# nmonette/TO-UED

Measured on AMD Instinct MI355X. Metric: agent-env-steps/sec (inner rollout) at num_agents=512; meta-updates/sec, higher is better.
Workload: dtype f32; 1 GPU; C2 LPG meta-gradient env_mode=tabular num_agents=512 num_mini_batches=1 W=64 T=20 K=5 score_function=random; num_agents=512, agents_per_gpu=512, env_workers=64, train_rollout_len=20, num_agent_updates=5, parallelism=dp1 (agent axis)

## Files before the change

### include/toued.h

```cpp
#ifndef TOUED_H
#define TOUED_H

#include <stddef.h>
#include <stdint.h>

#ifdef __cplusplus
extern "C" {
#endif

typedef struct ihipStream_t* hipStream_t;

typedef struct {
  int max_grid;
  int n_max;
  int n_types;
  int tabular;
} EnvSpec;

const char* toued_last_error(void);
int toued_abi_version(void);

typedef struct toued_ctx toued_ctx;
toued_ctx* toued_ctx_create(void);
int toued_ctx_destroy(toued_ctx* ctx);
// ... 27 lines not shown
                  int* obs_idx, int* obs_time, float* reward, uint8_t* done, int n, hipStream_t stream);

int toued_batch_reset(EnvSpec spec, const int* levels, const uint32_t* agent_keys, int n_agents, int W, int* state,
                      int* obs_idx, int* obs_time, hipStream_t stream);
int toued_batch_reset_masked(EnvSpec spec, const int* levels, const uint32_t* agent_keys, int n_agents, int W,
                             int* state, int* obs_idx, int* obs_time, const uint8_t* mask, hipStream_t stream);
int toued_rollout(EnvSpec spec, const int* levels, const float* theta, int D, const uint32_t* agent_keys,
                  int* state, int n_agents, int W, int T, int* traj_idx, int* traj_time, uint8_t* traj_action,
                  float* traj_reward, uint8_t* traj_done, float* cum_return, hipStream_t stream);
int toued_rollout_draws(EnvSpec spec, const int* levels, const uint32_t* keys, int n_agents, int U, int W, int T,
                        uint32_t* chain, uint32_t* draws, hipStream_t stream);
int toued_rollout_env(EnvSpec spec, const int* levels, const float* theta, int D, int* state, int n_agents, int W, int T,
                      const uint32_t* draws, long dstride, int* traj_idx, int* traj_time, uint8_t* traj_action,
                      float* traj_reward, uint8_t* traj_done, float* cum_return, hipStream_t stream);
int toued_eval_keys(const uint32_t* agent_keys, int n_agents, int W, int T, uint32_t* chain, hipStream_t stream);
int toued_eval_draws(EnvSpec spec, const int* levels, int n_agents, int W, int T, const uint32_t* chain,
                     uint32_t* draws, hipStream_t stream);
int toued_eval_returns(EnvSpec spec, const int* levels, const float* theta, int D, const int* state, int n_agents,
                       int W, int T, const uint32_t* draws, float* cum_return, hipStream_t stream);
int toued_eval_returns_cus(int n_workers);
int toued_optimal_return(const int* levels, int n, int max_grid, int n_max, int tabular, int max_rollout_len,
                         float* v0, float* v_all, hipStream_t stream);
int toued_policy_return(const int* levels, const float* theta, int n, int D, int max_grid, int n_max, int tabular,
                        int max_rollout_len, float* v0, float* v_all, hipStream_t stream);
int toued_policy_return_moments(const int* levels, const float* theta, int n, int D, int max_grid, int n_max,
                                int tabular, int max_rollout_len, float* v0, float* var0, float* v_all,
                                float* var_all, hipStream_t stream);


int toued_choice_cdf(const uint32_t* key, const float* cdf, int B, int n, int* out, hipStream_t stream);
// ... 165 lines not shown
                           float* d_y_hat, hipStream_t stream);

int toued_agent_step_snap(int N, int W, int T, int D, float* theta, float* phi, const int* tidx, const int* ttime,
                          const uint8_t* tact, const float* trew, const uint8_t* tdone, const float* pi_hat,
                          const float* y_hat, float alpha_y, float lr_a, float lr_c, float max_norm, float* Gth,
                          float* Gph, float* met, int* step, const int* levels, float* gstat, float* snap_th0,
                          float* snap_ph0, float* snap_last0, float* snap_th1, float* snap_ph1, float* snap_last1,
                          hipStream_t stream);
int toued_entropy_clip_hvp_snap(int N, int W, int T, int D, int K, const float* snap_th1, const float* snap_ph1,
                                const float* snap_last1, const float* snap_th0, const float* snap_ph0,
                                const float* snap_last0, const int* tidx, const int* ttime, const uint8_t* tact,
                                const float* pi_hat, const float* y_hat, float coef_a, float coef_c, float* adj_th,
                                float* adj_ph, const float* Gth, const float* Gph, const float* gstat, float lr_a,
                                float lr_c, float max_norm, float* coef, float alpha_y, float b2, float b3,
                                float* d_pi_hat, float* d_y_hat, hipStream_t stream);
int toued_embed_bwd_snap(int N, int W, int T, int D, int K, const float* snap_ph, const float* snap_last,
                         const int* ttime_hist, long tidx_stride, const uint8_t* tdone_hist, long tstep_stride,
                         const float* dX3, const float* dX4, long dx_stride_k, const float* e1w, const float* e1b,
                         const float* e2w, float* partial, int n_blocks, hipStream_t stream);

int toued_gru_pack_fwd_multi(const float* eta, long eta_stride, int n, const int* off, int F, float* fwdA,
                             hipStream_t stream);
int toued_gru_fwd_multi(int R, int T, int W, int F, int rows_per_cand, const float* X, long xs_f, long xs_col,
                        const uint8_t* done, const float* fwdA, const float* eta, long eta_stride, const int* off,
                        float* pi_hat, float* y_hat, hipStream_t stream);

int toued_es_ask(const uint32_t* key, long nd, long half_pop, long row_lo, long n_rows, const float* mean,
                 float sigma, float* x, hipStream_t stream);
int toued_es_grad(const float* x, const float* mean, float sigma, const float* fitness, int C, long nd, float* out,
                  hipStream_t stream);
// ... 8 lines not shown
```

### to-ued_amd/csrc/agent.hip

```cpp
#include <string.h>
#include <algorithm>
#include <type_traits>
#include "common.h"
#include "wave_dev.h"

#define EPSF 1e-8f
#define SORT_MAX_TW 2048

namespace {

TOUED_DEV float wave_sum(float v) {
#pragma unroll
  for (int o = 32; o > 0; o >>= 1) v += __shfl_xor(v, o, 64);
  return v;
}

template <int K>
TOUED_DEV void probs_of(const float* __restrict__ tab, const float* __restrict__ last, int idx, float c, float* p) {
  float l[K];
  float m = -__builtin_inff();
#pragma unroll
  for (int j = 0; j < K; ++j) {
    l[j] = *reinterpret_cast<const float*>(reinterpret_cast<const char*>(tab) + ((unsigned)idx * K + j) * 4u) + c * last[j];
    m = fmaxf(m, l[j]);
// ... 561 lines not shown
  }
  __syncthreads();
  if (tid == 0) {
    met[a * 8 + 3] += (red[0][0] + red[0][1]) + (red[0][2] + red[0][3]);
    met[a * 8 + 4] += (red[1][0] + red[1][1]) + (red[1][2] + red[1][3]);
  }
}

__global__ void __launch_bounds__(256) k_entropy_metric(int W, int T, int D, const float* __restrict__ theta,
                                                        const float* __restrict__ phi, const int* __restrict__ tidx,
                                                        const int* __restrict__ ttime, float* __restrict__ met) {
  __shared__ float red[2][4];
  entropy_metric_agent(blockIdx.x, threadIdx.x, W, T, D, theta, phi, tidx, ttime, met, red);
}

__global__ void __launch_bounds__(64) k_eval_loss(int N, int W, int T, int D, const float* __restrict__ theta,
                                                  const float* __restrict__ vcrit, const int* __restrict__ tidx,
                                                  const int* __restrict__ ttime, const uint8_t* __restrict__ tact,
                                                  const float* __restrict__ trew, const uint8_t* __restrict__ tdone,
                                                  float gamma, float lam, float* __restrict__ adv_scratch,
                                                  float* __restrict__ abar, float* __restrict__ out) {
  const int a = blockIdx.x;
  const int lane = threadIdx.x;
  const float* v = vcrit + (size_t)a * D;
  const float vlast = v[D - 1];
  const float* th = theta + (size_t)a * D * 5;
  float lastA[5];
#pragma unroll
  for (int j = 0; j < 5; ++j) lastA[j] = th[(size_t)(D - 1) * 5 + j];
  float* adv = adv_scratch + (size_t)a * W * T;
  float s_adv = 0.0f, s_vl = 0.0f;
  for (int w = lane; w < W; w += 64) {
    float vn = v[tidx[((size_t)a * (T + 1) + T) * W + w]] + ((float)ttime[((size_t)a * (T + 1) + T) * W + w] * 0.001f) * vlast;
    float g = 0.0f, vl = 0.0f;
    for (int t = T - 1; t >= 0; --t) {
      const size_t o0 = ((size_t)a * (T + 1) + t) * W + w;
// ... 1263 lines not shown
  if (ROWS_PRIO > 0) __builtin_amdgcn_s_setprio(ROWS_PRIO);
  rows_sorted_body<Op, false>(op);
}

#ifndef ROWS2_WPE
#define ROWS2_WPE 4
#endif
template <class Op1, class Op2>
__global__ void __launch_bounds__(512) __attribute__((amdgpu_waves_per_eu(ROWS2_WPE))) k_rows_sorted2(Op1 op1, Op2 op2) {
  if (ROWS_PRIO > 0) __builtin_amdgcn_s_setprio(ROWS_PRIO);
  rows_sorted_body<Op1, false, 1>(op1);
  __syncthreads();
  rows_sorted_body<Op2, true, 2>(op2);
}

template <class Op>
static bool launch_sorted(const Op& op, int N, hipStream_t stream) {
  const int TW = op.T * op.W;
  if (TW > SORT_MAX_TW || TW <= 0 || op.D >= (1 << 20)) return false;
  const size_t bytes = 2048 * 4 + (size_t)TW * (Op::NA + Op::NC) * 4;
  static bool attr_set = false;
  if (!attr_set) {
    if (hipFuncSetAttribute(reinterpret_cast<const void*>(&k_rows_sorted<Op>),
                            hipFuncAttributeMaxDynamicSharedMemorySize, 120 * 1024) != hipSuccess)
      return false;
    attr_set = true;
  }
  hipLaunchKernelGGL(k_rows_sorted<Op>, dim3(N), dim3(512), bytes, stream, op);
  return true;
}
// ... 264 lines not shown
      EntropyBwdOpT<true>{snap_th1, snap_ph1, tidx, ttime, coef_a, coef_c, adj_th, adj_ph, N, W, T, D, snap_last1};
  ec.Gth = Gth;
  ec.Gph = Gph;
  ec.gstat = gstat;
  ec.lr_a = lr_a;
  ec.lr_c = lr_c;
  ec.max_norm = max_norm;
  ec.coef = coef;
  const HvpOpT<true> hv{snap_th0, snap_ph0, tidx, ttime, tact, pi_hat, y_hat, Gth, Gph, adj_th, adj_ph, coef, lr_a,
                        lr_c, alpha_y, b2, b3, adj_th, adj_ph, d_pi_hat, d_y_hat, N, W, T, D, K, snap_last0};
  TOUED_REQUIRE(launch_sorted2(ec, hv, N, stream), "toued_entropy_clip_hvp_snap: cannot launch the sorted kernel");
  TOUED_CHECK_LAUNCH();
  return 0;
}

int toued_agent_apply(int N, int D, const float* th0, const float* ph0, const float* Gth, const float* Gph,
                      float lr_a, float lr_c, float max_norm, int* step, float* th1, float* ph1, const float* gstat,
                      hipStream_t stream) {
  if (N == 0 || D == 0) return 0;
  const bool v4 = aligned16(th0) && aligned16(ph0) && aligned16(Gth) && aligned16(Gph) && aligned16(th1) &&
                  aligned16(ph1);
  const long nvec = v4 ? (long)D * 2 + 1 : (long)D * 8;
  const unsigned gx = (unsigned)std::max(1L, std::min(64L, (nvec + 511) / 512));
  hipLaunchKernelGGL(k_agent_apply, dim3(gx, N, 2), dim3(256), 0, stream, N, D, th0, ph0, Gth, Gph, lr_a, lr_c,
                     max_norm, step, th1, ph1, gstat, v4 ? 1 : 0);
  TOUED_CHECK_LAUNCH();
  return 0;
}

int toued_entropy(int N, int W, int T, int D, const float* theta, const float* phi, const int* tidx, const int* ttime,
// ... 181 lines not shown
```

### to-ued_amd/csrc/env.hip

```cpp
#include "env_dev.h"

#include <cstdlib>
#include <cstring>

namespace {

template <int NMAX, bool TAB>
__global__ void __launch_bounds__(256) k_gw_reset(EnvSpec sp, const int* __restrict__ levels, int W,
                                                  const uint32_t* __restrict__ keys, int* __restrict__ state,
                                                  int* __restrict__ obs_idx, int* __restrict__ obs_time, int n) {
  const int i = blockIdx.x * blockDim.x + threadIdx.x;
  if (i >= n) return;
  const int* lev = levels + (size_t)(i / W) * LEVEL_WORDS;
  EnvState s;
  reset_env<NMAX, TAB>(sp, lev, make_uint2(keys[2 * i], keys[2 * i + 1]), s);
  store_state<NMAX>(state, n, i, s);
  obs_idx[i] = tab_index(sp, s);
  obs_time[i] = s.time;
}

template <int NMAX, bool TAB>
__global__ void __launch_bounds__(256) k_gw_step(EnvSpec sp, const int* __restrict__ levels, int W,
                                                 const uint32_t* __restrict__ keys, int* __restrict__ state,
                                                 const int* __restrict__ actions, int* __restrict__ obs_idx,
// ... 161 lines not shown

__global__ void __launch_bounds__(256) k_eval_keys(const uint32_t* __restrict__ agent_keys, int W, int T, int n,
                                                   uint4* __restrict__ chain) {
  const int i = blockIdx.x * blockDim.x + threadIdx.x;
  if (i >= n) return;
  const int a = i / W, w = i - a * W;
  uint2 r = split_at(make_uint2(agent_keys[2 * a], agent_keys[2 * a + 1]), (uint32_t)W, (uint32_t)w);
  for (int t = 0; t < T; ++t) {
    uint2 sub, sub_env;
    split2(r, r, sub);
    split2(r, r, sub_env);
    chain[(size_t)t * n + i] = make_uint4(sub.x, sub.y, sub_env.x, sub_env.y);
  }
}

__global__ void __launch_bounds__(1024) k_eval_keys_pairs(const uint32_t* __restrict__ agent_keys, int W, int T, int n,
                                                         uint2* __restrict__ chain) {
  const int g = blockIdx.x * blockDim.x + threadIdx.x;
  const int i = g >> 1;
  const uint32_t j = (uint32_t)(g & 1);
  if (i >= n) return;
  const int a = i / W, w = i - a * W;
  uint2 r = split_at(make_uint2(agent_keys[2 * a], agent_keys[2 * a + 1]), (uint32_t)W, (uint32_t)w);
  auto xor1 = [](uint32_t v) { return (uint32_t)__builtin_amdgcn_update_dpp(0, (int)v, 0xB1, 0xF, 0xF, false); };
  auto split_pair = [&](uint2& key, uint2& sub) {
    const uint2 y = threefry(key.x, key.y, j, j + 2u);
    const uint32_t px = xor1(y.x), py = xor1(y.y);
    key = j ? make_uint2(px, y.x) : make_uint2(y.x, px);
    sub = j ? make_uint2(py, y.y) : make_uint2(y.y, py);
  };
  for (int t = 0; t < T; ++t) {
    uint2 sub, sub_env;
    split_pair(r, sub);
    split_pair(r, sub_env);
    chain[((size_t)t * n + i) * 2 + j] = j ? sub_env : sub;
  }
}

template <int NMAX>
__global__ void __launch_bounds__(256) k_eval_draws(const int* __restrict__ levels, int W, int na, int n, long total,
                                                    const uint4* __restrict__ chain, uint4* __restrict__ draws) {
  const long j = (long)blockIdx.x * blockDim.x + threadIdx.x;
  if (j >= total) return;
  const int i = (int)(j % n);
  const int* lev = levels + (size_t)((i / W) % na) * LEVEL_WORDS;
  const uint4 c = chain[j];
  const draw4 d = step_draws<NMAX>(lev, make_uint2(c.x, c.y), make_uint2(c.z, c.w));
  draws[j] = make_uint4(d.x, d.y, d.z, d.w);
}

#ifdef H3_PLACE
// ... 124 lines not shown
    s.pos = pos;
    s.exists = (s.exists | (int)dr.z) & ~collected & used;
    s.early_term = term;
  }
  cum_return[i] = cum;
  if (EVAL_CHOSEN_ROW == 2 && warm == 1.2345e-38f) cum_return[i] = warm;
#ifdef H3_PLACE
  if (threadIdx.x == 0 && blockIdx.x < 64) {
    const unsigned slot = g_evr_launch & 63u;
    g_evr_place[(slot * 64 + blockIdx.x) * 2] = (unsigned)__builtin_amdgcn_s_getreg((3 << 11) | 20);
    g_evr_place[(slot * 64 + blockIdx.x) * 2 + 1] = (unsigned)__builtin_amdgcn_s_getreg((31 << 11) | 4);
  }
#endif
}

template <int NMAX, bool CAND>
__global__ void __launch_bounds__(256) k_train_env(EnvSpec sp, const int* __restrict__ levels,
                                                   const float* __restrict__ theta, int D, int* __restrict__ state,
                                                   int T, int W, int n, const uint4* __restrict__ draws, long dstride,
                                                   int* __restrict__ traj_idx, int* __restrict__ traj_time,
                                                   uint8_t* __restrict__ traj_action, float* __restrict__ traj_reward,
                                                   uint8_t* __restrict__ traj_done, float* __restrict__ cum_return) {
  const int i = blockIdx.x * blockDim.x + threadIdx.x;
  if (i >= n) return;
  const int a = i / W, w = i - a * W;
  const float* tab = theta + (size_t)a * D * 5;
  TrainWorker<NMAX, CAND> wk;
  wk.init(sp, levels, a, theta, D, state, n, i);
  wk.load_rows(tab, D);
  float cum = 0.0f, valid = 1.0f;
  const size_t base_o = (size_t)a * (T + 1) * W + w, base_t = (size_t)a * T * W + w;
  const draw4* dw = reinterpret_cast<const draw4*>(draws);
  draw4 dr0 = {0u, 0u, 0u, 0u};
  if (T > 0) dr0 = dw[i];
  draw4 dr1 = dr0;
  if (T > 1) dr1 = dw[dstride + i];
  for (int t = 0; t < T; ++t) {
// ... 85 lines not shown
  return 0;
}

int toued_batch_reset_masked(EnvSpec sp, const int* levels, const uint32_t* agent_keys, int n_agents, int W, int* state,
                             int* obs_idx, int* obs_time, const uint8_t* mask, hipStream_t stream) {
  if (int e = check_spec(sp)) return e;
  TOUED_REQUIRE(n_agents >= 0 && W >= 1 && mask, "toued_batch_reset_masked: bad sizes N=%d W=%d", n_agents, W);
  const int n = n_agents * W;
  if (n == 0) return 0;
  TOUED_DISPATCH(sp, hipLaunchKernelGGL((k_batch_reset<NMAX, TAB>), dim3(nblk(n)), dim3(256), 0, stream, sp, levels,
                                        agent_keys, W, state, obs_idx, obs_time, n, mask));
  TOUED_CHECK_LAUNCH();
  return 0;
}

int toued_eval_keys(const uint32_t* agent_keys, int n_agents, int W, int T, uint32_t* chain, hipStream_t stream) {
  TOUED_REQUIRE(n_agents >= 0 && W >= 1 && T >= 0, "toued_eval_keys: bad sizes N=%d W=%d T=%d", n_agents, W, T);
  const int n = n_agents * W;
  if (n == 0 || T == 0) return 0;
  static const int kb = [] {
    const char* e = getenv("TOUED_EVAL_KEYS_BLOCK");
    return e ? atoi(e) : 64;
  }();
  hipLaunchKernelGGL(k_eval_keys_pairs, dim3((unsigned)((2L * n + kb - 1) / kb)), dim3(kb), 0, stream, agent_keys, W, T,
                     n, reinterpret_cast<uint2*>(chain));
  TOUED_CHECK_LAUNCH();
  return 0;
}

int toued_eval_draws(EnvSpec sp, const int* levels, int n_agents, int W, int T, const uint32_t* chain, uint32_t* draws,
                     hipStream_t stream) {
  if (int e = check_spec(sp)) return e;
  TOUED_REQUIRE(sp.tabular, "toued_eval_draws: tabular envs only");
  TOUED_REQUIRE(n_agents >= 0 && W >= 1 && T >= 0, "toued_eval_draws: bad sizes N=%d W=%d T=%d", n_agents, W, T);
  const int n = n_agents * W;
  const long total = (long)n * T;
  if (total == 0) return 0;
  const unsigned g = (unsigned)((total + 255) / 256);
  TOUED_DISPATCH_NMAX(sp.n_max, true, hipLaunchKernelGGL(k_eval_draws<NMAX>, dim3(g), dim3(256), 0, stream, levels,
                                                        W, n_agents, n, total, reinterpret_cast<const uint4*>(chain),
                                                        reinterpret_cast<uint4*>(draws)));
  TOUED_CHECK_LAUNCH();
// ... 125 lines not shown
```

### to-ued_amd/toued/_lib.py

```python
from __future__ import annotations

import ctypes
import os
from pathlib import Path

import torch

LIB_PATH = Path(os.environ.get("TOUED_LIB", Path(__file__).resolve().parent / "libtoued_hip.so"))


class ToUEDError(RuntimeError):
    pass


class EnvSpecC(ctypes.Structure):
    _fields_ = [("max_grid", ctypes.c_int), ("n_max", ctypes.c_int), ("n_types", ctypes.c_int),
                ("tabular", ctypes.c_int)]


_P = ctypes.c_void_p
_I = ctypes.c_int
_F = ctypes.c_float
_U = ctypes.c_uint32
_L = ctypes.c_long
# ... 3 lines not shown
    "toued_split_planar": [_P, _I, _I, _P, _P],
    "toued_fold_in": [_P, _I, _U, _P, _P],
    "toued_random_bits": [_P, _I, _I, _P, _P],
    "toued_uniform": [_P, _I, _I, _F, _F, _P, _P],
    "toued_normal": [_P, _I, _I, _P, _P],
    "toued_mode_program_bytes": [],
    "toued_level_gen": [_P, _P, _P, _P, _P, _I, _P],
    "toued_level_gen_masked": [_P, _P, _P, _P, _I, _P, _P],
    "toued_level_edit": [_P, _P, _P, _I, _I, _I, _F, _I, _I, _F, _P, _P, _P],
    "toued_gw_reset": [EnvSpecC, _P, _I, _P, _P, _P, _P, _I, _P],
    "toued_gw_step": [EnvSpecC, _P, _I, _P, _P, _P, _P, _P, _P, _P, _I, _P],
    "toued_batch_reset": [EnvSpecC, _P, _P, _I, _I, _P, _P, _P, _P],
    "toued_batch_reset_masked": [EnvSpecC, _P, _P, _I, _I, _P, _P, _P, _P, _P],
    "toued_rollout": [EnvSpecC, _P, _P, _I, _P, _P, _I, _I, _I, _P, _P, _P, _P, _P, _P, _P],
    "toued_eval_keys": [_P, _I, _I, _I, _P, _P],
    "toued_rollout_draws": [EnvSpecC, _P, _P, _I, _I, _I, _I, _P, _P, _P],
    "toued_rollout_env": [EnvSpecC, _P, _P, _I, _P, _I, _I, _I, _P, _L, _P, _P, _P, _P, _P, _P, _P],
    "toued_eval_draws": [EnvSpecC, _P, _I, _I, _I, _P, _P, _P],
    "toued_eval_returns": [EnvSpecC, _P, _P, _I, _P, _I, _I, _I, _P, _P, _P],
    "toued_meta_keys": [_P, _I, _I, _P, _P, _P, _P, _P],
    "toued_lpg_inputs": [_I, _I, _I, _I, _I, _P, _P, _P, _P, _P, _P, _P, _P, _P, _P, _P, _P, _P, _P, _L, _L, _L, _P],
    "toued_lpg_inputs_rows": [_I, _I, _I, _I, _I, _P, _P, _P, _P, _P, _P, _P, _P, _P, _P, _P, _P, _P, _P, _L, _L, _L,
                              _P],
    "toued_agent_grad": [_I, _I, _I, _I, _P, _P, _P, _P, _P, _P, _P, _P, _P, _F, _P, _P, _P, _P, _P, _P, _P],
    "toued_agent_apply": [_I, _I, _P, _P, _P, _P, _F, _F, _F, _P, _P, _P, _P, _P],
    "toued_entropy": [_I, _I, _I, _I, _P, _P, _P, _P, _P, _F, _F, _P, _P, _P],
    "toued_eval_loss": [_I, _I, _I, _I, _P, _P, _P, _P, _P, _P, _P, _F, _F, _P, _P, _P, _P],
    "toued_lpgloss_grad": [_I, _I, _I, _I, _P, _P, _P, _P, _P, _P, _P],
    "toued_clip_dot": [_I, _I, _P, _P, _P, _P, _P, _F, _F, _F, _P, _P],
    "toued_hvp": [_I, _I, _I, _I, _I, _P, _P, _P, _P, _P, _P, _P, _P, _P, _P, _P, _P, _F, _F, _F, _F, _F,
# ... 27 lines not shown
    "toued_a2c_grad": [_I, _I, _I, _I, _P, _P, _P, _P, _P, _P, _P, _F, _F, _F, _P, _P, _P, _P],
    "toued_value_critic_update": [_I, _I, _I, _I, _P, _P, _P, _P, _P, _F, _F, _F, _F, _P, _P, _P],
    "toued_a2c_apply": [_I, _I, _P, _P, _P, _P, _F, _F, _F, _P, _P, _P],
    "toued_a2c_update_fits": [_I, _I, _I],
    "toued_a2c_update": [_I, _I, _I, _I, _P, _P, _P, _P, _P, _P, _P, _F, _F, _F, _F, _F, _F, _P, _P, _P, _P],
    "toued_agent_update_fits": [_I, _I, _I],
    "toued_agent_update": [_I, _I, _I, _I, _P, _P, _P, _P, _P, _P, _P, _P, _P, _F, _F, _F, _F, _P, _P, _P, _P, _P],
    "toued_agent_step": [_I, _I, _I, _I] + [_P] * 11 + [_F] * 4 + [_P] * 7,
    "toued_agent_step_entropy": [_I, _I, _I, _I] + [_P] * 11 + [_F] * 4 + [_P] * 7,
    "toued_gather_add": [_P, _P, _P, _P, _I, _P],
    "toued_sum_rows_add": [_P, _I, _I, _P, _P],
    "toued_sample_random_keys": [_P, _I, _I, _I, _P, _P, _P, _U, _P, _P, _P],
    "toued_entropy_clip_hvp": [_I] * 5 + [_P] * 9 + [_F] * 2 + [_P] * 5 + [_F] * 3 + [_P] + [_F] * 3 + [_P] * 3,
    "toued_agent_step_snap": [_I, _I, _I, _I] + [_P] * 9 + [_F] * 4 + [_P] * 13,
    "toued_entropy_clip_hvp_snap": [_I] * 5 + [_P] * 11 + [_F] * 2 + [_P] * 5 + [_F] * 3 + [_P] + [_F] * 3 + [_P] * 3,
    "toued_embed_bwd_snap": [_I] * 5 + [_P, _P, _P, _L, _P, _L, _P, _P, _L, _P, _P, _P, _P, _I, _P],
    "toued_meta_metrics": [_I, _I, _P, _F, _P, _F, _F, _F, _F, _P, _P],
    "toued_entropy_clip": [_I, _I, _I, _I, _P, _P, _P, _P, _F, _F, _P, _P, _P, _P, _P, _F, _F, _F, _P, _P],
    "toued_a2c_chain_fits": [_I, _I, _I],
    "toued_a2c_chain_self_fits": [_I, _I, _I],
    "toued_device_error_check": [_P, _I],
    "toued_sync_check": [],
    "toued_nonfinite_count": [_P, _L, _P, _P],
    "toued_nonfinite_count_2d": [_P, _L, _L, _L, _P, _P],
    "toued_dbg_wgrad_visits": [_P, _I],
    "toued_eval_returns_cus": [_I],
    "toued_optimal_return": [_P, _I, _I, _I, _I, _I, _P, _P, _P],
    "toued_policy_return": [_P, _P, _I, _I, _I, _I, _I, _I, _P, _P, _P],
    "toued_policy_return_moments": [_P, _P, _I, _I, _I, _I, _I, _I, _P, _P, _P, _P, _P],
    "toued_project_simplex": [_P, _P, _I, _I, _P, _P],
# ... 104 lines not shown
```

### to-ued_amd/toued/meta.py

```python
from __future__ import annotations

import os
from dataclasses import dataclass

import torch

from . import _lib, prng
from .agents import AgentBatch
from .debug import nan_checker
from .lpg import LPGGRU, LPGLayout, Y
from .rollout import RolloutWrapper, Transition, split_rollouts


@dataclass
class LpgHyperparams:
    num_agent_updates: int = 5
    agent_target_coeff: float = 0.5
    policy_entropy_coeff: float = 5e-2
    target_entropy_coeff: float = 1e-3
    policy_l2_coeff: float = 5e-3
    target_l2_coeff: float = 1e-3
    gamma: float = 0.99
    gae_lambda: float = 0.95
    actor_lr: float = 40.0
# ... 98 lines not shown
            raise ValueError(f"env_workers={W} must be a multiple of 32 for the MFMA GRU row blocks")
        self.R = R
        f32, i32, u8 = torch.float32, torch.int32, torch.uint8
        z = lambda *s, dt=f32: torch.zeros(s, dtype=dt, device=dev)
        self._ring = 0
        self._ring_last = 0
        self.G_th = z(K, N, D, 5)
        self.G_ph = z(K, N, D, Y)
        self.fused_step = (os.environ.get("TOUED_META_FUSED_STEP", "1") != "0"
                           and bool(_lib.lib().toued_agent_update_fits(W, T, D)))
        self.step_entropy = os.environ.get("TOUED_STEP_ENTROPY", "1") != "0"
        self.reverse_pair = os.environ.get("TOUED_REVERSE_PAIR", "1") != "0"
        self.hist_sparse = (os.environ.get("TOUED_HIST_SPARSE", "1") != "0" and self.fused_step
                            and self.step_entropy and self.reverse_pair
                            and os.environ.get("TOUED_HIST_RING", "1") != "0")
        if self.hist_sparse:
            self._theta_store = self._phi_store = None
            self.snap_th0, self.snap_th1 = z(K, N, T * W, 5), z(K, N, T * W, 5)
            self.snap_ph0, self.snap_ph1 = z(K, N, (T + 1) * W, Y), z(K, N, T * W, Y)
            self.snap_last0, self.snap_last1 = z(K, N, 16), z(K, N, 16)
            self._live = None
        else:
            self._theta_store = z(K + 1, N, D, 5)
            self._phi_store = z(K + 1, N, D, Y)
        self.gstat = z(K, N, 4)
        self.met = z(K, N, 8)
        self.traj = Transition(z(K + 1, N, T + 1, W, dt=i32), z(K + 1, N, T + 1, W, dt=i32),
                               z(K + 1, N, T, W, dt=u8), z(K + 1, N, T, W), z(K + 1, N, T, W, dt=u8))
        self.pi_hat = z(K, T, R)
        self.y_hat = z(K, T, Y, R)
# ... 8 lines not shown
        self.coef = z(N, 4)
        self.keys_train = z(K + 1, N, 2, dt=i32)
        self.keys_roll = self.keys_train[:K]
        self.keys_eval = self.keys_train[K]
        self.keys_ea_reset = z(N, 2, dt=i32)
        self.keys_ea_roll = z(N, 2, dt=i32)
        self.gru = LPGGRU(self.lay, R, T, K, W, dev)
        self.X = self.gru.X
        self.grad = z(self.lay.size)
        self.embed_blocks = 768
        self.embed_partial = z(self.embed_blocks, 161)
        self.ea_cum = None
        self.timers = KernelTimers()
        self.side = torch.cuda.Stream(device=dev)
        self._ea_draws = None
        self._draws = None

    @property
    def theta_h(self) -> torch.Tensor:
        if self.hist_sparse:
            return self._dense_history(0)
        return torch.roll(self._theta_store, -self._ring_last, dims=0)

    @property
    def phi_h(self) -> torch.Tensor:
        if self.hist_sparse:
            return self._dense_history(1)
        return torch.roll(self._phi_store, -self._ring_last, dims=0)

    def _dense_history(self, which: int) -> torch.Tensor:
# ... 52 lines not shown
        _lib.call("toued_adam", self.lay.size, _lib.ptr(eta), _lib.ptr(self.grad), _lib.ptr(adam.m), _lib.ptr(adam.v),
                  float(n_total), self.hyp.lpg_lr, 0.9, 0.999, 1e-8, adam.count, _lib.stream_ptr())
        nan_checker().check("eta_after_adam", eta)
        if len(parts) == 1:
            return parts[0]
        return _cat_metrics(parts)

    def _chunk(self, agent_keys: torch.Tensor, eta: torch.Tensor, agents):
        L = _lib
        N, W, T, K, D, R = self.N, self.W, self.T, self.K, self.D, self.R
        hyp = self.hyp
        st = L.stream_ptr()
        ptr = L.ptr
        L.call("toued_meta_keys", ptr(agent_keys), N, K, ptr(self.keys_roll), ptr(self.keys_eval),
               ptr(self.keys_ea_reset), ptr(self.keys_ea_roll), st)
        sparse = self.hist_sparse
        bound = not sparse and self.n_chunks == 1 and isinstance(agents, AgentBatch)
        ring = bound and os.environ.get("TOUED_HIST_RING", "1") != "0"
        r0 = self._ring if ring else 0
        if sparse:
            th = [agents.theta] * (K + 1)
            ph = [agents.phi] * (K + 1)
            self._live = (agents.theta, agents.phi)
        else:
            th = [self._theta_store[(r0 + k) % (K + 1)] for k in range(K + 1)]
            ph = [self._phi_store[(r0 + k) % (K + 1)] for k in range(K + 1)]
        self._ring_last = r0
        if sparse:
            if not (agents.theta.is_contiguous() and agents.phi.is_contiguous()):
                raise ValueError("MetaGradStep: the agents' tables must be contiguous (they are updated in place)")
# ... 9 lines not shown
        if not self.fused_step:
            self.G_th.zero_()
            self.G_ph.zero_()
        self.met.zero_()
        main = torch.cuda.current_stream()
        e1w, e1b = self._eta(eta, "e1_w"), self._eta(eta, "e1_b")
        e2w, e2b = self._eta(eta, "e2_w"), self._eta(eta, "e2_b")
        state = agents.state
        draws = None
        if split_rollouts():
            if self._draws is None:
                self._draws = tuple(torch.empty((T, (K + 1) * N * W, 4), dtype=torch.int32, device=self.dev)
                                    for _ in range(2))
            draws = self.ro.train_draws(self.keys_train, agents.levels, W,
                                        self._draws)
        ea = {}

        def start_eval_prep():
            self.side.wait_stream(main)
            with torch.cuda.stream(self.side):
                (_, _), ea["state"] = self.ro.batch_reset(self.keys_ea_reset, agents.levels, hyp.eval_workers)
                self._ea_draws = self.ro.eval_draws(self.keys_ea_roll, agents.levels, hyp.eval_workers,
                                                    self._ea_draws)
                ea["draws_done"] = torch.cuda.Event()
                ea["draws_done"].record(self.side)

        for k in range(K):
            tk = self._t(k)
            if self.fused_step and not sparse:
                self.side.wait_stream(main)
                with torch.cuda.stream(self.side):
                    th[k + 1].copy_(th[k])
                    ph[k + 1].copy_(ph[k])
                    copy_done = torch.cuda.Event()
                    copy_done.record(self.side)
            tok = self.timers.start("rollout")
            if draws is not None:
                self.ro.rollout_from_draws(draws, k, th[k], agents.levels, state, tk)
            else:
                self.ro.batch_rollout(self.keys_roll[k], th[k], agents.levels, state, out=tk,
                                      inplace_state=True)
            self.timers.stop(tok)
            nan_checker().check("rollout_rewards", tk.reward)
            L.call(lpg_inputs_fn(R, W), N, W, T, D, self.F, ptr(th[k]), ptr(ph[k]),
                   ptr(tk.obs_idx), ptr(tk.obs_time), ptr(tk.action), ptr(tk.reward), ptr(tk.done),
                   ptr(e1w), ptr(e1b), ptr(e2w), ptr(e2b), ptr(agents.step), ptr(agents.levels),
                   ptr(self.X) + 4 * k * T * R, self.gru.M, 1, 0, st)
            if k == 0:
                main.wait_event(self._packed)
            tok = self.timers.start("gru_fwd")
            self.gru.forward(k, self.X, tk.done, eta, self.pi_hat, self.y_hat)
            self.timers.stop(tok)
            if k == K - 1 and eval_keys_early() and eval_prep_after_forwards():
                start_eval_prep()
            if nan_checker().enabled:
                nan_checker().check("lpg_gru_states", self.gru.hin_block(k))
            nan_checker().check("lpg_outputs", self.pi_hat[k], self.y_hat[k])
            if sparse:
                L.call("toued_agent_step_snap", N, W, T, D, ptr(th[k]), ptr(ph[k]), ptr(tk.obs_idx), ptr(tk.obs_time),
                       ptr(tk.action), ptr(tk.reward), ptr(tk.done), ptr(self.pi_hat[k]), ptr(self.y_hat[k]),
                       hyp.agent_target_coeff, hyp.actor_lr, hyp.critic_lr, hyp.max_grad_norm, ptr(self.G_th[k]),
                       ptr(self.G_ph[k]), ptr(self.met[k]), ptr(agents.step), ptr(agents.levels), ptr(self.gstat[k]),
                       ptr(self.snap_th0[k]), ptr(self.snap_ph0[k]), ptr(self.snap_last0[k]), ptr(self.snap_th1[k]),
                       ptr(self.snap_ph1[k]), ptr(self.snap_last1[k]), st)
# ... 32 lines not shown
               ptr(te.obs_time), ptr(te.action), ptr(te.reward), ptr(te.done), hyp.gamma, hyp.gae_lambda,
               ptr(self.adv), ptr(self.abar), ptr(self.loss_out), st)
        if hyp.fix_value_critic:
            self._value_critic_update(te, agents)
        if not hyp.fix_value_critic:
            agents.vstep.add_(K + 1)
        key_cus = 2 * -(-N * hyp.eval_workers // 256)
        eval_cus = int(L.lib().toued_eval_returns_cus(N * hyp.eval_workers))

        def launch_eval():
            self.side.wait_stream(main)
            if "draws_done" not in ea:
                with torch.cuda.stream(self.side):
                    (_, _), ea["state"] = self.ro.batch_reset(self.keys_ea_reset, agents.levels, hyp.eval_workers)
                    self._ea_draws = self.ro.eval_draws(self.keys_ea_roll, agents.levels, hyp.eval_workers,
                                                        self._ea_draws)
                    ea["draws_done"] = torch.cuda.Event()
                    ea["draws_done"].record(self.side)
            ea["prev_reserve"] = L.lib().toued_set_reserved_cus(key_cus)

        def before_main_wgrad():
            small_done = torch.cuda.Event()
            small_done.record(main)
            self.side.wait_event(small_done)
            with torch.cuda.stream(self.side):
                ea["cum"] = self.ro.eval_returns_from_draws(self._ea_draws, th[K], agents.levels,
                                                            ea["state"])
            main.wait_event(ea["draws_done"])
            if os.environ.get("TOUED_EVAL_ALONE") == "1":
                main.wait_stream(self.side)
                return
            L.lib().toued_set_reserved_cus(eval_cus)
        if eval_keys_early() and "draws_done" not in ea:
            start_eval_prep()
        a_in = 0
        self.adj_th[a_in].zero_()
        self.adj_ph[a_in].zero_()
        L.call("toued_lpgloss_grad", N, W, T, D, ptr(th[K]), ptr(te.obs_idx), ptr(te.obs_time),
               ptr(te.action), ptr(self.abar), ptr(self.adj_th[a_in]), st)
        for k in range(K - 1, -1, -1):
            tk = self._t(k)
            if sparse:
                L.call("toued_entropy_clip_hvp_snap", N, W, T, D, K, ptr(self.snap_th1[k]), ptr(self.snap_ph1[k]),
                       ptr(self.snap_last1[k]), ptr(self.snap_th0[k]), ptr(self.snap_ph0[k]), ptr(self.snap_last0[k]),
                       ptr(tk.obs_idx), ptr(tk.obs_time), ptr(tk.action), ptr(self.pi_hat[k]), ptr(self.y_hat[k]),
                       -hyp.policy_entropy_coeff / K, -hyp.target_entropy_coeff / K, ptr(self.adj_th[a_in]),
                       ptr(self.adj_ph[a_in]), ptr(self.G_th[k]), ptr(self.G_ph[k]), ptr(self.gstat[k]), hyp.actor_lr,
                       hyp.critic_lr, hyp.max_grad_norm, ptr(self.coef), hyp.agent_target_coeff, hyp.policy_l2_coeff,
                       hyp.target_l2_coeff, ptr(self.d_pi_hat[k]), ptr(self.d_y_hat[k]), st)
                continue
            if self.fused_step and self.reverse_pair:
                L.call("toued_entropy_clip_hvp", N, W, T, D, K, ptr(th[k + 1]), ptr(ph[k + 1]),
                       ptr(th[k]), ptr(ph[k]), ptr(tk.obs_idx), ptr(tk.obs_time), ptr(tk.action),
                       ptr(self.pi_hat[k]), ptr(self.y_hat[k]), -hyp.policy_entropy_coeff / K,
                       -hyp.target_entropy_coeff / K, ptr(self.adj_th[a_in]), ptr(self.adj_ph[a_in]),
# ... 141 lines not shown
        gae_lambda=args.gae_lambda, actor_lr=ah.actor_learning_rate, critic_lr=ah.critic_learning_rate,
        max_grad_norm=ah.max_grad_norm, lpg_lr=args.lpg_learning_rate,
        fix_value_critic=bool(getattr(args, "fix_value_critic", False)))


def create_lpg_train_state(rng: torch.Tensor, args) -> LpgTrainState:
    from .lpg import flax_init_lpg_params
    eta = flax_init_lpg_params(rng, 7 if args.lifetime_conditioning else 5)
    return LpgTrainState(eta, None if args.use_es else AdamState(eta.numel(), eta.device))


def eval_prep_after_forwards() -> bool:
    return os.environ.get("TOUED_EVAL_PREP", "forwards") != "reverse"


def eval_keys_early() -> bool:
    return os.environ.get("TOUED_EVAL_KEYS_EARLY", "1") == "1"


def make_lpg_train_step(args, level_sampler, n_agents: int | None = None, world=None, rank_slice=None, impl=None):
    n_local = n_agents if n_agents is not None else (args.num_agents if rank_slice is None
                                                     else rank_slice[1] - rank_slice[0])
    holder = {} if impl is None else {"step": impl}
    if args.use_es:

        def es_step(rng, lpg_train_state, agent_states, value_critic_states=None):
            from .es import ESTrainStep
            if "step" not in holder:
                holder["step"] = ESTrainStep(args, level_sampler, n_local, lpg_train_state.params,
                                             lpg_train_state.params.device, world)
# ... 20 lines not shown
```

### to-ued_amd/toued/rollout.py

```python
from __future__ import annotations

import os

from dataclasses import dataclass

import numpy as np
import torch

from . import _lib
from .env import STATE_FIELDS, EnvSpec, get_env_spec


@dataclass
class Transition:
    obs_idx: torch.Tensor
    obs_time: torch.Tensor
    action: torch.Tensor
    reward: torch.Tensor
    done: torch.Tensor


def split_rollouts() -> bool:
    return os.environ.get("TOUED_ROLLOUT_FUSED") != "1"

# ... 94 lines not shown
            raise ValueError("train_draws: the buffers' worker stride must equal U * N * W")
        _lib.call("toued_rollout_draws", self._c, _lib.ptr(levels), _lib.ptr(keys.contiguous()), N, U, W, T,
                  _lib.ptr(chain), _lib.ptr(draws), stream if stream is not None else _lib.stream_ptr())
        return draws

    def rollout_from_draws(self, draws: torch.Tensor, u: int, theta: torch.Tensor, levels: torch.Tensor,
                           state: torch.Tensor, out: Transition, cum: torch.Tensor | None = None):
        N = theta.shape[0]
        n = state.shape[1]
        T = self.train_rollout_len
        _lib.call("toued_rollout_env", self._c, _lib.ptr(levels), _lib.ptr(theta), theta.shape[1], _lib.ptr(state), N,
                  n // N, T, _lib.ptr(draws) + 16 * u * n, draws.shape[1], _lib.ptr(out.obs_idx),
                  _lib.ptr(out.obs_time), _lib.ptr(out.action), _lib.ptr(out.reward), _lib.ptr(out.done),
                  _lib.ptr(cum) if cum is not None else None, _lib.stream_ptr())

    def eval_draws(self, agent_keys: torch.Tensor, levels: torch.Tensor, n_workers: int,
                   buf: torch.Tensor | None = None) -> torch.Tensor:
        N = agent_keys.shape[0]
        n, T = N * n_workers, self.eval_rollout_len
        dev = levels.device
        chain = torch.empty((T, n, 4), dtype=torch.int32, device=dev)
        if buf is None or buf.shape != (T, n, 4):
            buf = torch.empty((T, n, 4), dtype=torch.int32, device=dev)
        st = _lib.stream_ptr()
        _lib.call("toued_eval_keys", _lib.ptr(agent_keys.contiguous()), N, n_workers, T, _lib.ptr(chain), st)
        _lib.call("toued_eval_draws", self._c, _lib.ptr(levels), N, n_workers, T, _lib.ptr(chain), _lib.ptr(buf), st)
        return buf

    def eval_returns_from_draws(self, draws: torch.Tensor, theta: torch.Tensor, levels: torch.Tensor,
                                state: torch.Tensor) -> torch.Tensor:
        N = theta.shape[0]
        n = state.shape[1]
        cum = torch.empty((N, n // N), dtype=torch.float32, device=state.device)
        _lib.call("toued_eval_returns", self._c, _lib.ptr(levels), _lib.ptr(theta), theta.shape[1], _lib.ptr(state),
                  N, n // N, self.eval_rollout_len, _lib.ptr(draws), _lib.ptr(cum), _lib.stream_ptr())
        return cum

    def optimal_return(self, levels: torch.Tensor, max_rollout_len: int, return_all: bool = False) -> torch.Tensor:
        if not self.spec.tabular:
            raise NotImplementedError("Optimal return not implemented for non-tabular environments.")
        if levels.dim() == 1:
# ... 78 lines not shown
```

Measured before the change: 182.2 million agent-env-steps/sec.

## Split eval key generation across streams, fuse reverse loop kernel, raise wave priorities

Allows eval key/draw generation to be split into step ranges via a carry buffer, with an early piece launched on a separate stream, and reuses a persistent scratch buffer instead of allocating the chain each call. Adds an optional single fused kernel that runs the LPG loss gradient and the whole K-step entropy-clip/HVP reverse loop in one launch. Raises s_setprio on the eval-loss and train-env kernels so they win scheduling against concurrent side-stream work. The split defaults to zero and the fused reverse loop is off by default, so by default only the priority changes and the scratch reuse run.

Measured after the change: 182.7 million agent-env-steps/sec (median of 6 runs). No clear change (+0.3%).

```diff
diff --git a/include/toued.h b/include/toued.h
--- a/include/toued.h
+++ b/include/toued.h
@@ -65,6 +65,8 @@
                       const uint32_t* draws, long dstride, int* traj_idx, int* traj_time, uint8_t* traj_action,
                       float* traj_reward, uint8_t* traj_done, float* cum_return, hipStream_t stream);
 int toued_eval_keys(const uint32_t* agent_keys, int n_agents, int W, int T, uint32_t* chain, hipStream_t stream);
+int toued_eval_keys_range(const uint32_t* agent_keys, int n_agents, int W, int t0, int t1, uint32_t* carry,
+                          uint32_t* chain, hipStream_t stream);
 int toued_eval_draws(EnvSpec spec, const int* levels, int n_agents, int W, int T, const uint32_t* chain,
                      uint32_t* draws, hipStream_t stream);
 int toued_eval_returns(EnvSpec spec, const int* levels, const float* theta, int D, const int* state, int n_agents,
@@ -260,6 +262,14 @@
                                 float* adj_ph, const float* Gth, const float* Gph, const float* gstat, float lr_a,
                                 float lr_c, float max_norm, float* coef, float alpha_y, float b2, float b3,
                                 float* d_pi_hat, float* d_y_hat, hipStream_t stream);
+int toued_reverse_loop_snap(int N, int W, int T, int D, int K, const float* theta, const int* tidx_e,
+                            const int* ttime_e, const uint8_t* tact_e, const float* abar, const float* snap_th1,
+                            const float* snap_ph1, const float* snap_last1, const float* snap_th0,
+                            const float* snap_ph0, const float* snap_last0, const int* tidx, const int* ttime,
+                            const uint8_t* tact, const float* pi_hat, const float* y_hat, float coef_a, float coef_c,
+                            float* adj_th, float* adj_ph, const float* Gth, const float* Gph, const float* gstat,
+                            float lr_a, float lr_c, float max_norm, float* coef, float alpha_y, float b2, float b3,
+                            float* d_pi_hat, float* d_y_hat, hipStream_t stream);
 int toued_embed_bwd_snap(int N, int W, int T, int D, int K, const float* snap_ph, const float* snap_last,
                          const int* ttime_hist, long tidx_stride, const uint8_t* tdone_hist, long tstep_stride,
                          const float* dX3, const float* dX4, long dx_stride_k, const float* e1w, const float* e1b,
diff --git a/to-ued_amd/csrc/agent.hip b/to-ued_amd/csrc/agent.hip
--- a/to-ued_amd/csrc/agent.hip
+++ b/to-ued_amd/csrc/agent.hip
@@ -599,12 +599,16 @@
   entropy_metric_agent(blockIdx.x, threadIdx.x, W, T, D, theta, phi, tidx, ttime, met, red);
 }
 
+#ifndef EVAL_LOSS_PRIO
+#define EVAL_LOSS_PRIO 3
+#endif
 __global__ void __launch_bounds__(64) k_eval_loss(int N, int W, int T, int D, const float* __restrict__ theta,
                                                   const float* __restrict__ vcrit, const int* __restrict__ tidx,
                                                   const int* __restrict__ ttime, const uint8_t* __restrict__ tact,
                                                   const float* __restrict__ trew, const uint8_t* __restrict__ tdone,
                                                   float gamma, float lam, float* __restrict__ adv_scratch,
                                                   float* __restrict__ abar, float* __restrict__ out) {
+  if (EVAL_LOSS_PRIO > 0) __builtin_amdgcn_s_setprio(EVAL_LOSS_PRIO);
   const int a = blockIdx.x;
   const int lane = threadIdx.x;
   const float* v = vcrit + (size_t)a * D;
@@ -1898,6 +1902,45 @@
   rows_sorted_body<Op2, true, 2>(op2);
 }
 
+struct RevStrides {
+  size_t snap_a, snap_c0, snap_c1, last, tix, tact, pi, y, gth, gph, gstat;
+};
+__global__ void __launch_bounds__(512) __attribute__((amdgpu_waves_per_eu(4)))
+k_reverse_loop(LpgLossOp lpg, EntropyClipOpT<true> ec0, HvpOpT<true> hv0, RevStrides sd, int K) {
+  if (ROWS_PRIO > 0) __builtin_amdgcn_s_setprio(ROWS_PRIO);
+  rows_sorted_body<LpgLossOp, false, 1>(lpg);
+#pragma unroll 1
+  for (int k = K - 1; k >= 0; --k) {
+    const size_t uk = (size_t)k;
+    EntropyClipOpT<true> ec = ec0;
+    ec.theta += uk * sd.snap_a;
+    ec.phi += uk * sd.snap_c1;
+    ec.tlast += uk * sd.last;
+    ec.tidx += uk * sd.tix;
+    ec.ttime += uk * sd.tix;
+    ec.Gth += uk * sd.gth;
+    ec.Gph += uk * sd.gph;
+    ec.gstat += uk * sd.gstat;
+    __syncthreads();
+    rows_sorted_body<EntropyClipOpT<true>, false, 1>(ec);
+    HvpOpT<true> hv = hv0;
+    hv.theta += uk * sd.snap_a;
+    hv.phi += uk * sd.snap_c0;
+    hv.tlast += uk * sd.last;
+    hv.tidx += uk * sd.tix;
+    hv.ttime += uk * sd.tix;
+    hv.tact += uk * sd.tact;
+    hv.pi_hat += uk * sd.pi;
+    hv.y_hat += uk * sd.y;
+    hv.Gth += uk * sd.gth;
+    hv.Gph += uk * sd.gph;
+    hv.d_pi_hat += uk * sd.pi;
+    hv.d_y_hat += uk * sd.y;
+    __syncthreads();
+    rows_sorted_body<HvpOpT<true>, true, 2>(hv);
+  }
+}
+
 template <class Op>
 static bool launch_sorted(const Op& op, int N, hipStream_t stream) {
   const int TW = op.T * op.W;
@@ -2192,6 +2235,49 @@
   return 0;
 }
 
+int toued_reverse_loop_snap(int N, int W, int T, int D, int K, const float* theta, const int* tidx_e,
+                            const int* ttime_e, const uint8_t* tact_e, const float* abar, const float* snap_th1,
+                            const float* snap_ph1, const float* snap_last1, const float* snap_th0,
+                            const float* snap_ph0, const float* snap_last0, const int* tidx, const int* ttime,
+                            const uint8_t* tact, const float* pi_hat, const float* y_hat, float coef_a, float coef_c,
+                            float* adj_th, float* adj_ph, const float* Gth, const float* Gph, const float* gstat,
+                            float lr_a, float lr_c, float max_norm, float* coef, float alpha_y, float b2, float b3,
+                            float* d_pi_hat, float* d_y_hat, hipStream_t stream) {
+  TOUED_REQUIRE(K >= 1, "toued_reverse_loop_snap: K=%d", K);
+  TOUED_REQUIRE(toued_agent_update_fits(W, T, D), "toued_reverse_loop_snap: W=%d T=%d D=%d unsupported", W, T, D);
+  TOUED_REQUIRE(hvp_offsets_fit(N, W, T), "toued_reverse_loop_snap: 32*N*T*W = %ld bytes exceed the 32-bit offsets",
+                32L * N * T * W);
+  TOUED_REQUIRE(snap_th1 && snap_ph1 && snap_last1 && snap_th0 && snap_ph0 && snap_last0,
+                "toued_reverse_loop_snap: every snapshot is required");
+  if (N == 0) return 0;
+  const LpgLossOp lpg{theta, tidx_e, ttime_e, tact_e, abar, adj_th, N, W, T, D};
+  EntropyClipOpT<true> ec;
+  static_cast<EntropyBwdOpT<true>&>(ec) =
+      EntropyBwdOpT<true>{snap_th1, snap_ph1, tidx, ttime, coef_a, coef_c, adj_th, adj_ph, N, W, T, D, snap_last1};
+  ec.Gth = Gth;
+  ec.Gph = Gph;
+  ec.gstat = gstat;
+  ec.lr_a = lr_a;
+  ec.lr_c = lr_c;
+  ec.max_norm = max_norm;
+  ec.coef = coef;
+  const HvpOpT<true> hv{snap_th0, snap_ph0, tidx, ttime, tact, pi_hat, y_hat, Gth, Gph, adj_th, adj_ph, coef, lr_a,
+                        lr_c, alpha_y, b2, b3, adj_th, adj_ph, d_pi_hat, d_y_hat, N, W, T, D, K, snap_last0};
+  const size_t S = (size_t)N * T * W, NW = (size_t)N * W, ND = (size_t)N * D;
+  const RevStrides sd{5 * S, 8 * (S + NW), 8 * S, 16 * (size_t)N, S + NW, S, S, 8 * S, 5 * ND, 8 * ND, 4 * (size_t)N};
+  const size_t bytes = 2048 * 4 + (size_t)T * W * 13 * 4;
+  static bool attr_set = false;
+  if (!attr_set) {
+    TOUED_REQUIRE(hipFuncSetAttribute(reinterpret_cast<const void*>(&k_reverse_loop),
+                                      hipFuncAttributeMaxDynamicSharedMemorySize, 120 * 1024) == hipSuccess,
+                  "toued_reverse_loop_snap: cannot launch the sorted kernel");
+    attr_set = true;
+  }
+  hipLaunchKernelGGL(k_reverse_loop, dim3(N), dim3(512), bytes, stream, lpg, ec, hv, sd, K);
+  TOUED_CHECK_LAUNCH();
+  return 0;
+}
+
 int toued_agent_apply(int N, int D, const float* th0, const float* ph0, const float* Gth, const float* Gph,
                       float lr_a, float lr_c, float max_norm, int* step, float* th1, float* ph1, const float* gstat,
                       hipStream_t stream) {
diff --git a/to-ued_amd/csrc/env.hip b/to-ued_amd/csrc/env.hip
--- a/to-ued_amd/csrc/env.hip
+++ b/to-ued_amd/csrc/env.hip
@@ -199,14 +199,17 @@
   }
 }
 
-__global__ void __launch_bounds__(1024) k_eval_keys_pairs(const uint32_t* __restrict__ agent_keys, int W, int T, int n,
+__global__ void __launch_bounds__(1024) k_eval_keys_pairs(const uint32_t* __restrict__ agent_keys, int W, int t0,
+                                                         int t1, int n, uint32_t* carry,
                                                          uint2* __restrict__ chain) {
   const int g = blockIdx.x * blockDim.x + threadIdx.x;
   const int i = g >> 1;
   const uint32_t j = (uint32_t)(g & 1);
   if (i >= n) return;
   const int a = i / W, w = i - a * W;
-  uint2 r = split_at(make_uint2(agent_keys[2 * a], agent_keys[2 * a + 1]), (uint32_t)W, (uint32_t)w);
+  uint2 r;
+  if (t0 == 0) r = split_at(make_uint2(agent_keys[2 * a], agent_keys[2 * a + 1]), (uint32_t)W, (uint32_t)w);
+  else r = make_uint2(carry[2 * (size_t)i], carry[2 * (size_t)i + 1]);
   auto xor1 = [](uint32_t v) { return (uint32_t)__builtin_amdgcn_update_dpp(0, (int)v, 0xB1, 0xF, 0xF, false); };
   auto split_pair = [&](uint2& key, uint2& sub) {
     const uint2 y = threefry(key.x, key.y, j, j + 2u);
@@ -214,12 +217,13 @@
     key = j ? make_uint2(px, y.x) : make_uint2(y.x, px);
     sub = j ? make_uint2(py, y.y) : make_uint2(y.y, py);
   };
-  for (int t = 0; t < T; ++t) {
+  for (int t = t0; t < t1; ++t) {
     uint2 sub, sub_env;
     split_pair(r, sub);
     split_pair(r, sub_env);
     chain[((size_t)t * n + i) * 2 + j] = j ? sub_env : sub;
   }
+  if (carry) carry[2 * (size_t)i + j] = j ? r.y : r.x;
 }
 
 template <int NMAX>
@@ -374,6 +378,9 @@
 #endif
 }
 
+#ifndef TRAIN_ENV_PRIO
+#define TRAIN_ENV_PRIO 3
+#endif
 template <int NMAX, bool CAND>
 __global__ void __launch_bounds__(256) k_train_env(EnvSpec sp, const int* __restrict__ levels,
                                                    const float* __restrict__ theta, int D, int* __restrict__ state,
@@ -381,6 +388,7 @@
                                                    int* __restrict__ traj_idx, int* __restrict__ traj_time,
                                                    uint8_t* __restrict__ traj_action, float* __restrict__ traj_reward,
                                                    uint8_t* __restrict__ traj_done, float* __restrict__ cum_return) {
+  if (TRAIN_ENV_PRIO > 0) __builtin_amdgcn_s_setprio(TRAIN_ENV_PRIO);
   const int i = blockIdx.x * blockDim.x + threadIdx.x;
   if (i >= n) return;
   const int a = i / W, w = i - a * W;
@@ -496,18 +504,33 @@
   return 0;
 }
 
-int toued_eval_keys(const uint32_t* agent_keys, int n_agents, int W, int T, uint32_t* chain, hipStream_t stream) {
-  TOUED_REQUIRE(n_agents >= 0 && W >= 1 && T >= 0, "toued_eval_keys: bad sizes N=%d W=%d T=%d", n_agents, W, T);
+static int eval_keys_range(const uint32_t* agent_keys, int n_agents, int W, int t0, int t1, uint32_t* carry,
+                           uint32_t* chain, hipStream_t stream) {
   const int n = n_agents * W;
-  if (n == 0 || T == 0) return 0;
+  if (n == 0) return 0;
   static const int kb = [] {
     const char* e = getenv("TOUED_EVAL_KEYS_BLOCK");
     return e ? atoi(e) : 64;
   }();
-  hipLaunchKernelGGL(k_eval_keys_pairs, dim3((unsigned)((2L * n + kb - 1) / kb)), dim3(kb), 0, stream, agent_keys, W, T,
-                     n, reinterpret_cast<uint2*>(chain));
-  TOUED_CHECK_LAUNCH();
-  return 0;
+  hipLaunchKernelGGL(k_eval_keys_pairs, dim3((unsigned)((2L * n + kb - 1) / kb)), dim3(kb), 0, stream, agent_keys, W,
+                     t0, t1, n, carry, reinterpret_cast<uint2*>(chain));
+  TOUED_CHECK_LAUNCH();
+  return 0;
+}
+
+int toued_eval_keys(const uint32_t* agent_keys, int n_agents, int W, int T, uint32_t* chain, hipStream_t stream) {
+  TOUED_REQUIRE(n_agents >= 0 && W >= 1 && T >= 0, "toued_eval_keys: bad sizes N=%d W=%d T=%d", n_agents, W, T);
+  if (T == 0) return 0;
+  return eval_keys_range(agent_keys, n_agents, W, 0, T, nullptr, chain, stream);
+}
+
+int toued_eval_keys_range(const uint32_t* agent_keys, int n_agents, int W, int t0, int t1, uint32_t* carry,
+                          uint32_t* chain, hipStream_t stream) {
+  TOUED_REQUIRE(n_agents >= 0 && W >= 1 && 0 <= t0 && t0 <= t1,
+                "toued_eval_keys_range: bad sizes N=%d W=%d t0=%d t1=%d", n_agents, W, t0, t1);
+  TOUED_REQUIRE(carry, "toued_eval_keys_range: carry is required");
+  if (t0 == t1 && t0 > 0) return 0;
+  return eval_keys_range(agent_keys, n_agents, W, t0, t1, carry, chain, stream);
 }
 
 int toued_eval_draws(EnvSpec sp, const int* levels, int n_agents, int W, int T, const uint32_t* chain, uint32_t* draws,
diff --git a/to-ued_amd/toued/_lib.py b/to-ued_amd/toued/_lib.py
--- a/to-ued_amd/toued/_lib.py
+++ b/to-ued_amd/toued/_lib.py
@@ -41,6 +41,7 @@
     "toued_batch_reset_masked": [EnvSpecC, _P, _P, _I, _I, _P, _P, _P, _P, _P],
     "toued_rollout": [EnvSpecC, _P, _P, _I, _P, _P, _I, _I, _I, _P, _P, _P, _P, _P, _P, _P],
     "toued_eval_keys": [_P, _I, _I, _I, _P, _P],
+    "toued_eval_keys_range": [_P, _I, _I, _I, _I, _P, _P, _P],
     "toued_rollout_draws": [EnvSpecC, _P, _P, _I, _I, _I, _I, _P, _P, _P],
     "toued_rollout_env": [EnvSpecC, _P, _P, _I, _P, _I, _I, _I, _P, _L, _P, _P, _P, _P, _P, _P, _P],
     "toued_eval_draws": [EnvSpecC, _P, _I, _I, _I, _P, _P, _P],
@@ -98,6 +99,7 @@
     "toued_entropy_clip_hvp": [_I] * 5 + [_P] * 9 + [_F] * 2 + [_P] * 5 + [_F] * 3 + [_P] + [_F] * 3 + [_P] * 3,
     "toued_agent_step_snap": [_I, _I, _I, _I] + [_P] * 9 + [_F] * 4 + [_P] * 13,
     "toued_entropy_clip_hvp_snap": [_I] * 5 + [_P] * 11 + [_F] * 2 + [_P] * 5 + [_F] * 3 + [_P] + [_F] * 3 + [_P] * 3,
+    "toued_reverse_loop_snap": [_I] * 5 + [_P] * 16 + [_F] * 2 + [_P] * 5 + [_F] * 3 + [_P] + [_F] * 3 + [_P] * 3,
     "toued_embed_bwd_snap": [_I] * 5 + [_P, _P, _P, _L, _P, _L, _P, _P, _L, _P, _P, _P, _P, _I, _P],
     "toued_meta_metrics": [_I, _I, _P, _F, _P, _F, _F, _F, _F, _P, _P],
     "toued_entropy_clip": [_I, _I, _I, _I, _P, _P, _P, _P, _F, _F, _P, _P, _P, _P, _P, _F, _F, _F, _P, _P],
diff --git a/to-ued_amd/toued/meta.py b/to-ued_amd/toued/meta.py
--- a/to-ued_amd/toued/meta.py
+++ b/to-ued_amd/toued/meta.py
@@ -136,6 +136,7 @@
         self.hist_sparse = (os.environ.get("TOUED_HIST_SPARSE", "1") != "0" and self.fused_step
                             and self.step_entropy and self.reverse_pair
                             and os.environ.get("TOUED_HIST_RING", "1") != "0")
+        self.reverse_fused = os.environ.get("TOUED_REVERSE_FUSED", "0") == "1" and self.K >= 1
         if self.hist_sparse:
             self._theta_store = self._phi_store = None
             self.snap_th0, self.snap_th1 = z(K, N, T * W, 5), z(K, N, T * W, 5)
@@ -174,6 +175,10 @@
         self.timers = KernelTimers()
         self.side = torch.cuda.Stream(device=dev)
         self._ea_draws = None
+        self._ea_scratch = None
+        self.eval_keys_split = max(0, min(int(os.environ.get("TOUED_EVAL_KEYS_SPLIT", eval_keys_split_default())),
+                                          rollout.eval_rollout_len))
+        self.early = torch.cuda.Stream(device=dev)
         self._draws = None
 
     @property
@@ -256,6 +261,18 @@
         ptr = L.ptr
         L.call("toued_meta_keys", ptr(agent_keys), N, K, ptr(self.keys_roll), ptr(self.keys_eval),
                ptr(self.keys_ea_reset), ptr(self.keys_ea_roll), st)
+        ea = {}
+        main = torch.cuda.current_stream()
+        if self._ea_scratch is None:
+            self._ea_scratch = self.ro.eval_draws_scratch(N, hyp.eval_workers, self.dev)
+        T1 = self.eval_keys_split if eval_keys_early() else 0
+        if T1 > 0:
+            self.early.wait_stream(main)
+            with torch.cuda.stream(self.early):
+                self._ea_draws = self.ro.eval_draws(self.keys_ea_roll, agents.levels, hyp.eval_workers,
+                                                    self._ea_draws, self._ea_scratch, (0, T1))
+                ea["early_done"] = torch.cuda.Event()
+                ea["early_done"].record(self.early)
         sparse = self.hist_sparse
         bound = not sparse and self.n_chunks == 1 and isinstance(agents, AgentBatch)
         ring = bound and os.environ.get("TOUED_HIST_RING", "1") != "0"
@@ -295,14 +312,16 @@
                                     for _ in range(2))
             draws = self.ro.train_draws(self.keys_train, agents.levels, W,
                                         self._draws)
-        ea = {}
 
         def start_eval_prep():
             self.side.wait_stream(main)
+            if "early_done" in ea:
+                self.side.wait_event(ea["early_done"])
             with torch.cuda.stream(self.side):
                 (_, _), ea["state"] = self.ro.batch_reset(self.keys_ea_reset, agents.levels, hyp.eval_workers)
                 self._ea_draws = self.ro.eval_draws(self.keys_ea_roll, agents.levels, hyp.eval_workers,
-                                                    self._ea_draws)
+                                                    self._ea_draws, self._ea_scratch,
+                                                    (T1, self.ro.eval_rollout_len))
                 ea["draws_done"] = torch.cuda.Event()
                 ea["draws_done"].record(self.side)
 
@@ -329,6 +348,8 @@
                    ptr(self.X) + 4 * k * T * R, self.gru.M, 1, 0, st)
             if k == 0:
                 main.wait_event(self._packed)
+                if "early_done" in ea:
+                    main.wait_event(ea["early_done"])
             tok = self.timers.start("gru_fwd")
             self.gru.forward(k, self.X, tk.done, eta, self.pi_hat, self.y_hat)
             self.timers.stop(tok)
@@ -391,7 +412,7 @@
                 with torch.cuda.stream(self.side):
                     (_, _), ea["state"] = self.ro.batch_reset(self.keys_ea_reset, agents.levels, hyp.eval_workers)
                     self._ea_draws = self.ro.eval_draws(self.keys_ea_roll, agents.levels, hyp.eval_workers,
-                                                        self._ea_draws)
+                                                        self._ea_draws, self._ea_scratch)
                     ea["draws_done"] = torch.cuda.Event()
                     ea["draws_done"].record(self.side)
             ea["prev_reserve"] = L.lib().toued_set_reserved_cus(key_cus)
@@ -413,9 +434,21 @@
         a_in = 0
         self.adj_th[a_in].zero_()
         self.adj_ph[a_in].zero_()
-        L.call("toued_lpgloss_grad", N, W, T, D, ptr(th[K]), ptr(te.obs_idx), ptr(te.obs_time),
-               ptr(te.action), ptr(self.abar), ptr(self.adj_th[a_in]), st)
-        for k in range(K - 1, -1, -1):
+        fused = sparse and self.reverse_fused
+        if fused:
+            tr = self.traj
+            L.call("toued_reverse_loop_snap", N, W, T, D, K, ptr(th[K]), ptr(te.obs_idx), ptr(te.obs_time),
+                   ptr(te.action), ptr(self.abar), ptr(self.snap_th1), ptr(self.snap_ph1), ptr(self.snap_last1),
+                   ptr(self.snap_th0), ptr(self.snap_ph0), ptr(self.snap_last0), ptr(tr.obs_idx), ptr(tr.obs_time),
+                   ptr(tr.action), ptr(self.pi_hat), ptr(self.y_hat), -hyp.policy_entropy_coeff / K,
+                   -hyp.target_entropy_coeff / K, ptr(self.adj_th[a_in]), ptr(self.adj_ph[a_in]), ptr(self.G_th),
+                   ptr(self.G_ph), ptr(self.gstat), hyp.actor_lr, hyp.critic_lr, hyp.max_grad_norm, ptr(self.coef),
+                   hyp.agent_target_coeff, hyp.policy_l2_coeff, hyp.target_l2_coeff, ptr(self.d_pi_hat),
+                   ptr(self.d_y_hat), st)
+        else:
+            L.call("toued_lpgloss_grad", N, W, T, D, ptr(th[K]), ptr(te.obs_idx), ptr(te.obs_time),
+                   ptr(te.action), ptr(self.abar), ptr(self.adj_th[a_in]), st)
+        for k in () if fused else range(K - 1, -1, -1):
             tk = self._t(k)
             if sparse:
                 L.call("toued_entropy_clip_hvp_snap", N, W, T, D, K, ptr(self.snap_th1[k]), ptr(self.snap_ph1[k]),
@@ -587,6 +620,10 @@
     return os.environ.get("TOUED_EVAL_PREP", "forwards") != "reverse"
 
 
+def eval_keys_split_default() -> int:
+    return 0
+
+
 def eval_keys_early() -> bool:
     return os.environ.get("TOUED_EVAL_KEYS_EARLY", "1") == "1"
 
diff --git a/to-ued_amd/toued/rollout.py b/to-ued_amd/toued/rollout.py
--- a/to-ued_amd/toued/rollout.py
+++ b/to-ued_amd/toued/rollout.py
@@ -132,17 +132,40 @@
                   _lib.ptr(out.obs_time), _lib.ptr(out.action), _lib.ptr(out.reward), _lib.ptr(out.done),
                   _lib.ptr(cum) if cum is not None else None, _lib.stream_ptr())
 
+    def eval_draws_scratch(self, n_agents: int, n_workers: int, device) -> tuple[torch.Tensor, torch.Tensor]:
+        n, T = n_agents * n_workers, self.eval_rollout_len
+        return (torch.empty((T, n, 4), dtype=torch.int32, device=device),
+                torch.empty((n, 2), dtype=torch.int32, device=device))
+
     def eval_draws(self, agent_keys: torch.Tensor, levels: torch.Tensor, n_workers: int,
-                   buf: torch.Tensor | None = None) -> torch.Tensor:
+                   buf: torch.Tensor | None = None, scratch: tuple[torch.Tensor, torch.Tensor] | None = None,
+                   steps: tuple[int, int] | None = None) -> torch.Tensor:
         N = agent_keys.shape[0]
         n, T = N * n_workers, self.eval_rollout_len
         dev = levels.device
-        chain = torch.empty((T, n, 4), dtype=torch.int32, device=dev)
         if buf is None or buf.shape != (T, n, 4):
+            if steps is not None and steps[0] > 0:
+                raise ValueError("eval_draws: a later piece needs the buffer its first piece returned")
             buf = torch.empty((T, n, 4), dtype=torch.int32, device=dev)
         st = _lib.stream_ptr()
-        _lib.call("toued_eval_keys", _lib.ptr(agent_keys.contiguous()), N, n_workers, T, _lib.ptr(chain), st)
-        _lib.call("toued_eval_draws", self._c, _lib.ptr(levels), N, n_workers, T, _lib.ptr(chain), _lib.ptr(buf), st)
+        if scratch is None:
+            if steps is not None:
+                raise ValueError("eval_draws: steps needs a scratch kept between the pieces (eval_draws_scratch)")
+            chain = torch.empty((T, n, 4), dtype=torch.int32, device=dev)
+            _lib.call("toued_eval_keys", _lib.ptr(agent_keys.contiguous()), N, n_workers, T, _lib.ptr(chain), st)
+            t0, t1 = 0, T
+        else:
+            chain, carry = scratch
+            if chain.shape != (T, n, 4) or carry.shape != (n, 2):
+                raise ValueError(f"eval_draws: scratch {tuple(chain.shape)}, {tuple(carry.shape)} for T={T}, "
+                                 f"{n} workers")
+            t0, t1 = (0, T) if steps is None else steps
+            if not 0 <= t0 <= t1 <= T:
+                raise ValueError(f"eval_draws: steps {steps} outside [0, {T}]")
+            _lib.call("toued_eval_keys_range", _lib.ptr(agent_keys.contiguous()), N, n_workers, t0, t1, _lib.ptr(carry),
+                      _lib.ptr(chain), st)
+        _lib.call("toued_eval_draws", self._c, _lib.ptr(levels), N, n_workers, t1 - t0, _lib.ptr(chain) + 16 * n * t0,
+                  _lib.ptr(buf) + 16 * n * t0, st)
         return buf
 
     def eval_returns_from_draws(self, draws: torch.Tensor, theta: torch.Tensor, levels: torch.Tensor,
```
